# auggiemarignier/pxmcmc

Measured on AMD Instinct MI355X. Metric: MYULA samples/sec at L=256 synthesis, higher is better.
Workload: dtype f64

## Files before the change

include/pxmcmc_amd.h:

```cpp
#ifndef PXMCMC_AMD_H
#define PXMCMC_AMD_H

#include <stddef.h>
#include <stdint.h>

#ifdef __cplusplus
extern "C" {
#endif

typedef struct pxm_sht_plan_s* pxm_sht_plan_t;
typedef struct pxm_wav_plan_s* pxm_wav_plan_t;
typedef struct pxm_dwav_plan_s* pxm_dwav_plan_t;
typedef struct pxm_hwav_plan_s* pxm_hwav_plan_t;
typedef void* pxm_stream_t;

int pxm_version(void);
#ifdef PXM_NOISE_F64
#error "the -DPXM_NOISE_F64 build switch was removed: pass the flag PXM_NOISE_F64 per call (one library serves both precisions)"
#endif
#define PXM_NOISE_F64 16
int pxm_noise_bits(void);
int64_t pxm_host_check_address_ranges(int L, double B, int J_min, int spin, int max_chains, int what);
const char* pxm_last_error(void);
int pxm_device_count(void);

int pxm_capture_begin(void);
int pxm_capture_end(void);
int pxm_deferred_pending(void);
int pxm_tables_trim(void);

int pxm_j_max(int L, double B);
int pxm_wav_bandlimits(int L, double B, int J_min, int* bl_out, int cap);
int64_t pxm_wav_ncoefs(int L, double B, int J_min, int64_t* nscal_out);
int pxm_tiling_axisym(int L, double B, int J_min, double* kappa0, double* kappa);
int pxm_mw_ring_weights(int L, double* q);
int pxm_host_sht_tables(int L, int spin, int m, double* Binv, double* Afwd);
int pxm_host_rec_table(int L, int spin, int m, double* Brec);
int pxm_host_pfa511_tables(uint16_t* idx, double* b2);

int pxm_sht_plan_create(int L, int spin, int max_chains, unsigned flags, pxm_sht_plan_t* plan);
int pxm_sht_plan_destroy(pxm_sht_plan_t plan);
int pxm_sht_uses_recursion(pxm_sht_plan_t plan);
int pxm_rec_reduce_selftest(double* out128);
int pxm_sht_inverse(pxm_sht_plan_t plan, const void* flm, void* f, int C, pxm_stream_t stream);
int pxm_sht_forward(pxm_sht_plan_t plan, const void* f, void* flm, int C, pxm_stream_t stream);
// ... 170 lines not shown
```

pxmcmc_amd/_lib.py:

```python
import ctypes as C
import os

import torch

_HERE = os.path.dirname(os.path.abspath(__file__))
LIB_PATH = os.environ.get("PXM_LIB_PATH") or os.path.join(_HERE, "lib", "libpxmcmc_amd.so")

c_i64, c_u64, c_int, c_dbl, c_vp = C.c_int64, C.c_uint64, C.c_int, C.c_double, C.c_void_p

SIGNATURES = {
    "pxm_version": (c_int, []),
    "pxm_noise_bits": (c_int, []),
    "pxm_host_check_address_ranges": (c_i64, [c_int, c_dbl, c_int, c_int, c_int, c_int]),
    "pxm_last_error": (C.c_char_p, []),
    "pxm_device_count": (c_int, []),
    "pxm_capture_begin": (c_int, []),
    "pxm_capture_end": (c_int, []),
    "pxm_deferred_pending": (c_int, []),
    "pxm_tables_trim": (c_int, []),
    "pxm_wav_set_iter_counter": (c_int, [c_vp, c_vp]),
    "pxm_wav_release_iter_counter": (c_int, [c_vp, c_vp]),
    "pxm_wav_iter_counter_add": (c_int, [c_vp, c_u64, c_vp]),
    "pxm_wav_exact_dft_scales": (c_int, [c_vp]),
    "pxm_wav_status": (c_int, [c_vp, c_int, c_vp]),
    "pxm_sht_status": (c_int, [c_vp, c_int, c_vp]),
    "pxm_wav_profile_enable": (c_int, [c_vp, c_int]),
    "pxm_wav_profile_read": (c_int, [c_vp, c_vp, c_vp, c_vp, c_vp]),
    "pxm_wav_profile_read_launches": (c_int, [c_vp, c_vp, c_vp, c_vp, c_i64, c_vp]),
    "pxm_wav_profile_read_dft": (c_int, [c_vp, c_vp, c_vp, c_vp]),
    "pxm_wav_workspace_nonfinite": (c_i64, [c_vp, c_vp]),
    "pxm_reduce_scratch_doubles": (c_i64, [c_int]),
    "pxm_j_max": (c_int, [c_int, c_dbl]),
    "pxm_wav_bandlimits": (c_int, [c_int, c_dbl, c_int, c_vp, c_int]),
    "pxm_wav_ncoefs": (c_i64, [c_int, c_dbl, c_int, c_vp]),
    "pxm_tiling_axisym": (c_int, [c_int, c_dbl, c_int, c_vp, c_vp]),
    "pxm_mw_ring_weights": (c_int, [c_int, c_vp]),
# ... 159 lines not shown
```

pxmcmc_amd/csrc/sht_core.h:

```cpp
#pragma once
#include "common.h"

namespace pxm {

enum TableKind { TAB_INV = 0, TAB_FWD = 1, TAB_INV_ADJ = 2, TAB_FWD_ADJ = 3, TAB_GRAM = 4, TAB_KINDS = 5 };
inline bool kind_el_to_ring(int kind) { return kind == TAB_INV || kind == TAB_FWD_ADJ; }
inline bool kind_rows_are_el(int kind) { return kind == TAB_FWD || kind == TAB_INV_ADJ || kind == TAB_GRAM; }
inline bool kind_k_is_el(int kind) { return kind == TAB_INV || kind == TAB_FWD_ADJ || kind == TAB_GRAM; }

struct GemmTask {
  int64_t tab_off;
  int64_t rt_stride;
  int64_t x_off[4];
  int64_t y_off[4];
  int64_t x2_off[4];
  int64_t hd_off[4];
  int64_t ks_off[2];
  int64_t rs_off[2];
  int row_lo[2], row_hi[2];
  int k_beg, k_end;
  int row0;
  int n_rt;
  int nslab;
  double sign1;
  int m_unit;
  int hd_stride;
  int x_ncol, y_ncol;
};

struct GemmAffine {
  double ns = 0, wr = 0, wi = 0;
// ... 22 lines not shown
    p.launch_bytes.push_back(alg_bytes);
    p.launch_wgs.push_back(workgroups);
    ++p.used;
  }
};
int profiler_enable(Profiler* pr, int max_launches);
int profiler_read(Profiler::Pool* p, double* ms, int64_t* launches, double* bytes, double* flops,
                  double* per_launch_ms = nullptr, double* per_launch_bytes = nullptr, int64_t cap = 0,
                  int32_t* per_launch_wgs = nullptr);
void profiler_release(Profiler* pr);

struct GemmFuse {
  int64_t x2_base = -1;
  const double* rscale = nullptr;
  int row_lo = 0, row_hi = 1 << 30;
  int64_t hd_base = -1;
  int hd_stride = 0;
};

struct ShtTables {
  int L = 0, spin = 0, Rp = 0;
  bool paired = false;
  int n_m = 0;
  double* d_tab[TAB_KINDS] = {nullptr, nullptr, nullptr, nullptr, nullptr};
  size_t bytes[TAB_KINDS] = {0, 0, 0, 0, 0};
  std::vector<int64_t> m_off[TAB_KINDS];
  std::vector<int> k_beg[TAB_KINDS];
  int refs = 0;
  int m_of(int i) const { return paired ? i : i - (L - 1); }
};

int get_tables(int L, int spin, unsigned kinds_mask, ShtTables** out);
void retain_tables(ShtTables* T);
void release_tables(ShtTables* T);
int64_t tables_trim();

void append_gemm_tasks(const ShtTables& T, int kind, int ncol, int64_t x_base, int x_L, int x_Rp,
                       int64_t y_base, int y_L, int y_Rp, const double* kscale, int64_t scratch_off,
                       const double* ws_base, std::vector<GemmTask>& tasks, int el_lo = 0,
                       const GemmFuse& fuse = GemmFuse());
struct GemmSide {
  int64_t x_base, y_base;
  int x_L, x_Rp, y_L, y_Rp;
  const double* kscale;
  int el_lo;
  GemmFuse fuse;
  int x_ncol = 0, y_ncol = 0;
};

void append_gemm_tasks_packed(const ShtTables& T, int kind, int ncol, const GemmSide& side_a, const GemmSide* side_b,
                              int64_t scratch_off, const double* ws_base, std::vector<GemmTask>& tasks);
int launch_gemm_packed(const GemmTask* d_tasks, int n_tasks, int pk, int flags, const double* X, double* Y, int ncol, int col0,
                       double alg_bytes, double flops, hipStream_t stream, Profiler* prof = nullptr);
// ... 121 lines not shown
```

pxmcmc_amd/csrc/sht_gemm.hip:

```cpp
#include "../../include/pxmcmc_amd.h"
#include "sht_core.h"

#include <type_traits>

#include <hip/hip_ext.h>

#include <cstdlib>
#include <map>
#include <mutex>

namespace pxm {

typedef double d4 __attribute__((ext_vector_type(4)));

constexpr int KC = 16;
#define PXM_GEMM_MFMA(ACC, A, B) ACC = __builtin_amdgcn_mfma_f64_16x16x4f64(A, B, ACC, 0, 0, 0);
#ifdef PXM_GEMM_TRACE
__device__ unsigned long long* g_gemm_trace = nullptr;
extern "C" int pxm_debug_set_gemm_trace(unsigned long long* buf) {
  return hipMemcpyToSymbol(HIP_SYMBOL(g_gemm_trace), &buf, sizeof(buf)) == hipSuccess ? 0 : -1;
}
#endif
__device__ __forceinline__ double stage_add(double a, double b, bool on) { return a + (on ? b : 0.0); }
__device__ __forceinline__ double2 stage_add(double2 a, double2 b, bool on) { return double2{a.x + (on ? b.x : 0.0), a.y + (on ? b.y : 0.0)}; }
__device__ __forceinline__ double stage_scale(double a, double sc) { return a * sc; }
__device__ __forceinline__ double2 stage_scale(double2 a, double sc) { return double2{a.x * sc, a.y * sc}; }
template <int CT, int NSLAB>
struct GemmGeom {
  static constexpr int NCT = CT * NSLAB;
  static constexpr int COLS = 16 * NCT;
  static constexpr int PITCH = COLS + (COLS == 16 ? 0 : 16);
};
template <int CT, int NSLAB, int NW, int RT, int NSET, bool TWO, bool SK, int PK = 0>
__device__ __forceinline__ void sht_gemm_body(const GemmTask* __restrict__ tasks, const int bid,
                                              const double* __restrict__ X, double* __restrict__ Y, int ncol, int col0,
                                              const GemmAffine& aff, double (*xs)[KC][GemmGeom<CT, NSLAB>::PITCH]) {
  constexpr int NCT = CT * NSLAB;
  constexpr bool HOIST = TWO;
  constexpr int COLS = GemmGeom<CT, NSLAB>::COLS;
  constexpr int PITCH = GemmGeom<CT, NSLAB>::PITCH;
  constexpr int NT = 64 * NW;
  constexpr int VW = (KC * COLS / 2 >= NT) ? 2 : 1;
  constexpr int NV = KC * COLS / VW;
  constexpr int IT = (NV + NT - 1) / NT;
  const GemmTask t = tasks[bid];
  const int tid = threadIdx.x, lane = tid & 63;
  if (t.n_rt == 0) return;
  const int xn = PK ? t.x_ncol : ncol, yn = PK ? t.y_ncol : ncol;
#ifdef PXM_GEMM_TRACE
  const unsigned long long trace_t0 = wall_clock64();
  unsigned long long trace_t1 = 0, trace_t2 = 0;
  long long trace_c[5] = {0, 0, 0, 0, 0};
#define PXM_GEMM_CSTAMP(K) if (ch == 8) trace_c[K] = clock64();
#else
#define PXM_GEMM_CSTAMP(K)
#endif
  const int wave = __builtin_amdgcn_readfirstlane(tid >> 6);
  const int kq = lane >> 4, cl = lane & 15;
  const int n_my = min(RT, max(0, t.n_rt - RT * wave));
  const int nch = (t.k_end - t.k_beg) / KC;

  const double* sp[IT];
  const double* sp2[IT];
  const double* skp[IT];
  int so[IT];
  bool sv[IT];
#pragma unroll
  for (int i = 0; i < IT; ++i) {
    const int q0 = tid + NT * i;
    const int q = q0 % NV;
    const int kr = (q / (COLS / VW)) % KC, col = VW * (q % (COLS / VW));
// ... 140 lines not shown
    const int64_t yo = tasks[bid].y_off[live ? slab : 0];
    const int row_lo = grp ? t.row_lo[1] : t.row_lo[0], row_hi = grp ? t.row_hi[1] : t.row_hi[0];
#pragma unroll
    for (int r = 0; r < RT; ++r) {
      if (r >= n_my) continue;
      const int rowb = t.row0 + 16 * (RT * wave + r) + kq;
      double* yb = Y + yo + col0 + (cl % PK) + (int64_t)rowb * yn;
#pragma unroll
      for (int q = 0; q < 4; ++q) {
        const int row = rowb + 4 * q;
        const double rs = grp ? rsv[r][NGRP - 1][q] : rsv[r][0][q];
        if (live && row >= row_lo && row < row_hi) yb[(int64_t)(4 * q) * yn] = sgn * rs * acc[r][0][q];
      }
    }
  } else {
#pragma unroll
  for (int r = 0; r < RT; ++r) {
    if (r >= n_my) continue;
#pragma unroll
    for (int c = 0; c < NCT; ++c) {
      const int slab = c / CT, cin = 16 * (c % CT), grp = slab >> 1;
      const double sgn = (slab & 1) ? t.sign1 : 1.0;
      const int rowb = t.row0 + 16 * (RT * wave + r) + kq;
      double* yb = Y + t.y_off[slab] + col0 + cin + cl + (int64_t)rowb * ncol;
#pragma unroll
      for (int q = 0; q < 4; ++q) {
        const int row = rowb + 4 * q;
        double v = acc[r][c][q];
        if (aff.on) {
          const double u = aff.ns * v - hdv[r][slab][q];
          int lo = __double2loint(u), hi = __double2hiint(u);
          lo = __builtin_amdgcn_mov_dpp(lo, 0xB1, 0xF, 0xF, true);
          hi = __builtin_amdgcn_mov_dpp(hi, 0xB1, 0xF, 0xF, true);
          const double pu = __hiloint2double(hi, lo);
          v = (cl & 1) ? (aff.wr * u + aff.wi * pu) : (aff.wr * u - aff.wi * pu);
          if (col0 + cin + cl >= aff.ncol_live) v = 0.0;
        }
        if (row >= t.row_lo[grp] && row < t.row_hi[grp]) yb[(int64_t)(4 * q) * ncol] = sgn * rsv[r][grp][q] * v;
      }
    }
  }
  }
#ifdef PXM_GEMM_TRACE
  __syncthreads();
  if (tid == 0 && g_gemm_trace) {
    unsigned hw, xcc;
    asm volatile("s_getreg_b32 %0, hwreg(HW_REG_HW_ID)" : "=s"(hw));
    asm volatile("s_getreg_b32 %0, hwreg(HW_REG_XCC_ID)" : "=s"(xcc));
    const unsigned long long slot = atomicAdd(g_gemm_trace, 1ull);
    unsigned long long* r = g_gemm_trace + 8 + 8 * slot;
    r[0] = blockIdx.x; r[1] = gridDim.x; r[2] = trace_t0; r[3] = wall_clock64();
    r[4] = ((unsigned long long)(xcc & 0xf) << 32) | hw; r[5] = (unsigned long long)nch | ((unsigned long long)t.n_rt << 16) | ((unsigned long long)aff.on << 32);
    r[6] = trace_t1; r[7] = trace_t2;
    if (nch > 9) {
      const unsigned long long s2 = atomicAdd(g_gemm_trace + 1, 1ull);
      unsigned long long* q = g_gemm_trace + 8 + 8 * 8192 + 8 * s2;
      q[0] = nch; q[1] = trace_c[1] - trace_c[0]; q[2] = trace_c[2] - trace_c[1]; q[3] = trace_c[3] - trace_c[2];
      q[4] = trace_c[4] - trace_c[3]; q[5] = aff.on; q[6] = gridDim.x; q[7] = 0;
    }
  }
#endif
// ... 70 lines not shown
int check_gemm_task_ranges(const std::vector<GemmTask>& v, int nslab, int flags, int ncol, const double* ws_base,
                           const char* list_name) {
  int64_t n = 0;
  std::string why;
  auto bad = [&](size_t ti, const char* what, int col0) {
    set_error(std::string("GEMM task address range outside its buffer: list '") + list_name + "', task " + std::to_string(ti) +
              ", column group " + std::to_string(col0) + ", " + what + ": " + why);
    return -1;
  };
  auto ok = [&](int64_t lo, int64_t hi) {
    ++n;
    return lo <= hi && dev_range_ok(ws_base + lo, ws_base + hi + 1, &why);
  };
  const bool TWO = flags & 1, SK = flags & 2;
  for (size_t ti = 0; ti < v.size(); ++ti) {
    const GemmTask& t = v[ti];
    if (t.n_rt == 0) continue;
    const int nch = (t.k_end - t.k_beg) / KC;
    if (!ok(t.tab_off, t.tab_off + (int64_t)(t.n_rt - 1) * t.rt_stride + (int64_t)(2 * (nch - 1) + 1) * 128 + 127))
      return bad(ti, "ring-table stream", 0);
    for (int col0 = 0; col0 < ncol; col0 += 32) {
      const int CT = (ncol - col0 >= 32) ? 2 : 1;
      for (int slab = 0; slab < nslab; ++slab) {
        const int xn = t.x_ncol ? t.x_ncol : ncol, yn = t.y_ncol ? t.y_ncol : ncol;
        const int wx = std::min(16 * CT, xn), wy = std::min(16 * CT, yn);
        const int64_t lo = col0 + (int64_t)t.k_beg * xn, hi = col0 + wx - 1 + (int64_t)(t.k_end - 1) * xn;
        if (!ok(t.x_off[slab] + lo, t.x_off[slab] + hi)) return bad(ti, "operand staging", col0);
        if (TWO && t.x2_off[slab] && !ok(t.x2_off[slab] + lo, t.x2_off[slab] + hi)) return bad(ti, "second operand staging", col0);
        if (SK && t.ks_off[slab >> 1] && !ok(t.ks_off[slab >> 1] + t.k_beg, t.ks_off[slab >> 1] + t.k_end - 1))
          return bad(ti, "operand scale vector", col0);
        const int64_t r_lo = t.row0, r_hi = t.row0 + 16 * t.n_rt - 1;
        if (t.hd_off[slab] && !ok(t.hd_off[slab] + r_lo * t.hd_stride, t.hd_off[slab] + r_hi * t.hd_stride + 1))
          return bad(ti, "affine data term", col0);
        if (t.rs_off[slab >> 1] && !ok(t.rs_off[slab >> 1] + r_lo, t.rs_off[slab >> 1] + r_hi))
          return bad(ti, "per-row output scale", col0);
        const int64_t s_lo = std::max<int64_t>(r_lo, t.row_lo[slab >> 1]), s_hi = std::min<int64_t>(r_hi, (int64_t)t.row_hi[slab >> 1] - 1);
        if (s_lo <= s_hi && !ok(t.y_off[slab] + col0 + s_lo * yn, t.y_off[slab] + col0 + wy - 1 + s_hi * yn))
          return bad(ti, "result rows", col0);
      }
    }
  }
  ranges_checked_add(n);
  return 0;
}

int gemm_rows_per_task(int ncol) {
  (void)ncol;
// ... 67 lines not shown
    }
  } else {
    g.x_off[s1] = g.x_off[s0];
    g.y_off[s1] = g.y_off[s0];
  }
  g.ks_off[grp] = sd.kscale ? (sd.kscale - ws_base) : 0;
  g.rs_off[grp] = sd.fuse.rscale ? (sd.fuse.rscale - ws_base) : 0;
  g.row_lo[grp] = sd.fuse.row_lo;
  g.row_hi[grp] = sd.fuse.row_hi;
  g.x2_off[s0] = g.x2_off[s1] = 0;
  if (sd.fuse.x2_base >= 0) {
    g.x2_off[s0] = sd.fuse.x2_base + (int64_t)(m + sd.x_L - 1) * sd.x_Rp * xn;
    g.x2_off[s1] = (T.paired && m != 0) ? sd.fuse.x2_base + (int64_t)(-m + sd.x_L - 1) * sd.x_Rp * xn : g.x2_off[s0];
  }
  g.hd_off[s0] = g.hd_off[s1] = 0;
  g.hd_stride = sd.fuse.hd_stride > 0 ? sd.fuse.hd_stride : ncol;
  if (sd.fuse.hd_base >= 0) {
    g.hd_off[s0] = sd.fuse.hd_base + (int64_t)(m + sd.y_L - 1) * sd.y_Rp * g.hd_stride;
    g.hd_off[s1] = (T.paired && m != 0) ? sd.fuse.hd_base + (int64_t)(-m + sd.y_L - 1) * sd.y_Rp * g.hd_stride : g.hd_off[s0];
  }
  (void)kind;
}

static void append_tasks_impl(const ShtTables& T, int kind, int ncol, const GemmSide& side,
                              int64_t scratch_off, const double* ws_base, std::vector<GemmTask>& tasks) {
  const bool rows_el = kind_rows_are_el(kind), k_el = kind_k_is_el(kind);
  const int Rp = T.Rp;
  const int el_lo = side.el_lo;
  const int lo16 = round_down(std::max(el_lo, 0), 16);
  const int rpt = gemm_rows_per_task(ncol);
  for (int i = 0; i < T.n_m; ++i) {
    const int m = T.m_of(i);
    const int kb = T.k_beg[kind][i];
    const int start = std::max(kb, lo16);
    if (start >= Rp) continue;
    const int64_t rt_stride = (int64_t)((k_el ? Rp - kb : Rp) / 8) * 128;
    const int k_beg = k_el ? start : 0, k_end = Rp, row_beg = rows_el ? start : 0;
    const int64_t tab_skip = (rows_el ? (int64_t)((start - kb) / 16) * rt_stride : 0) + (k_el ? (int64_t)((start - kb) / 8) * 128 : 0);
    const int n_rt_total = (Rp - row_beg) / 16;
    for (int rt = 0; rt < n_rt_total; rt += rpt) {
      GemmTask g;
      g.m_unit = T.paired ? m : m + T.L - 1;
      g.tab_off = (T.d_tab[kind] + T.m_off[kind][i] + tab_skip + (int64_t)rt * rt_stride) - ws_base;
      g.rt_stride = rt_stride;
      for (int s = 0; s < 2; ++s) fill_side(g, s, T, kind, m, ncol, side, scratch_off, ws_base);
      g.nslab = T.paired ? 2 : 1;
      g.k_beg = k_beg;
      g.k_end = k_end;
      g.row0 = row_beg + 16 * rt;
      g.n_rt = std::min(rpt, n_rt_total - rt);
      g.sign1 = (kind == TAB_GRAM) ? 1.0 : ((m & 1) ? -1.0 : 1.0);
      g.x_ncol = side.x_ncol ? side.x_ncol : ncol;
      g.y_ncol = side.y_ncol ? side.y_ncol : ncol;
      tasks.push_back(g);
    }
  }
}

void append_gemm_tasks_packed(const ShtTables& T, int kind, int ncol, const GemmSide& side_a, const GemmSide* side_b,
                              int64_t scratch_off, const double* ws_base, std::vector<GemmTask>& tasks) {
  GemmSide sa = side_a;
  if (side_b) sa.el_lo = std::min(side_a.el_lo, side_b->el_lo);
  const size_t first = tasks.size();
  append_tasks_impl(T, kind, ncol, sa, scratch_off, ws_base, tasks);
  for (size_t i = first; i < tasks.size(); ++i) {
    GemmTask& g = tasks[i];
    const int m = T.paired ? g.m_unit : g.m_unit - (T.L - 1);
    fill_side(g, 0, T, kind, m, ncol, side_a, scratch_off, ws_base);
    fill_side(g, 1, T, kind, m, ncol, side_b ? *side_b : side_a, scratch_off, ws_base);
    g.nslab = side_b ? 4 : 2;
    g.x_ncol = side_a.x_ncol ? side_a.x_ncol : ncol;
    g.y_ncol = side_a.y_ncol ? side_a.y_ncol : ncol;
    if (!T.paired) {
      g.nslab = 1;
    }
  }
}
// ... 7 lines not shown

__global__ void k_build_fwd(const double* __restrict__ Bd, const double* __restrict__ Qd, double* __restrict__ Ad,
                            int Rp, int L, double scale, int m0, int spin) {
  const int i = blockIdx.z;
  const int el = blockIdx.x * 16 + threadIdx.x, t = blockIdx.y * 16 + threadIdx.y;
  const int m = m0 + i;
  const int par = ((m + spin) & 1) ? 1 : 0;
  const double* B = Bd + (int64_t)i * Rp * Rp;
  const double* Q = Qd + (int64_t)par * Rp * Rp;
  double acc = 0;
  for (int tp = 0; tp < L; ++tp) acc += B[(int64_t)tp * Rp + el] * Q[(int64_t)tp * Rp + t];
  Ad[(int64_t)i * Rp * Rp + (int64_t)el * Rp + t] = scale * acc;
}

__global__ void k_build_gram(const double* __restrict__ Bd, double* __restrict__ Gd, int Rp, int L) {
  const int i = blockIdx.z;
  const int r = blockIdx.x * 16 + threadIdx.x, c = blockIdx.y * 16 + threadIdx.y;
  const double* B = Bd + (int64_t)i * Rp * Rp;
  double acc = 0;
  for (int t = 0; t < L; ++t) acc += B[(int64_t)t * Rp + r] * B[(int64_t)t * Rp + c];
  Gd[(int64_t)i * Rp * Rp + (int64_t)r * Rp + c] = acc;
}

__global__ void k_tile_table(const double* __restrict__ D, double* __restrict__ out, int Rp, int row_beg,
                             int k_beg, int transposed) {
  const int nk2 = (Rp - k_beg) / 8;
  const int rt = blockIdx.y;
  const int kk2 = blockIdx.x;
  const int lane = threadIdx.x >> 1, h = threadIdx.x & 1;
  const int row = row_beg + 16 * rt + (lane & 15);
  const int k = k_beg + 8 * kk2 + 4 * h + (lane >> 4);
  const double v = transposed ? D[(int64_t)k * Rp + row] : D[(int64_t)row * Rp + k];
  out[((int64_t)rt * nk2 + kk2) * 128 + threadIdx.x] = v;
}

static std::mutex g_tab_mutex;
static std::map<std::pair<int, int>, ShtTables*> g_tab_cache;

static int build_kind(ShtTables& T, int kind, const double* d_B, const double* d_A, const double* d_G) {
  const int Rp = T.Rp;
  const bool rows_el = kind_rows_are_el(kind), k_el = kind_k_is_el(kind);
  T.m_off[kind].resize(T.n_m);
  T.k_beg[kind].resize(T.n_m);
  int64_t total = 0;
  for (int i = 0; i < T.n_m; ++i) {
    const int elmin = std::max(std::abs(T.m_of(i)), std::abs(T.spin));
    const int kb = round_down(elmin, 16);
    T.k_beg[kind][i] = kb;
    T.m_off[kind][i] = total;
    total += (int64_t)((rows_el ? Rp - kb : Rp) / 16) * ((k_el ? Rp - kb : Rp) / 8) * 128;
  }
  T.bytes[kind] = (size_t)total * sizeof(double);
  if (int rc = dev_alloc(&T.d_tab[kind], T.bytes[kind], "ring table")) return rc;
  if (dry_run()) return 0;
  for (int i = 0; i < T.n_m; ++i) {
    const int kb = T.k_beg[kind][i];
    const double* src;
    int transposed;
    if (kind == TAB_INV) { src = d_B; transposed = 0; }
    else if (kind == TAB_FWD_ADJ) { src = d_A; transposed = 1; }
    else if (kind == TAB_FWD) { src = d_A; transposed = 0; }
    else if (kind == TAB_INV_ADJ) { src = d_B; transposed = 1; }
    else { src = d_G; transposed = 0; }
    src += (int64_t)i * Rp * Rp;
    const int row_beg = rows_el ? kb : 0, k_beg = k_el ? kb : 0;
    dim3 grid((Rp - k_beg) / 8, (Rp - row_beg) / 16), block(128);
    if (grid.x == 0 || grid.y == 0) continue;
    hipLaunchKernelGGL(k_tile_table, grid, block, 0, 0, src, T.d_tab[kind] + T.m_off[kind][i], Rp, row_beg, k_beg,
                       transposed);
  }
  PXM_HIP(hipGetLastError());
  return 0;
}

int get_tables(int L, int spin, unsigned kinds_mask, ShtTables** out) {
  std::lock_guard<std::mutex> lock(g_tab_mutex);
  int dev = 15;
  if (!dry_run()) {
    PXM_HIP(hipGetDevice(&dev));
    PXM_REQUIRE(dev >= 0 && dev < 15, "get_tables: device index outside [0, 15)");
  }
  auto key = std::make_pair(L * 16 + dev, spin);
  ShtTables* T = nullptr;
  auto it = g_tab_cache.find(key);
  if (it != g_tab_cache.end()) T = it->second;
  else {
    T = new ShtTables();
    T->L = L;
    T->spin = spin;
    T->Rp = round_up(L, 16);
    T->paired = (spin == 0);
    T->n_m = T->paired ? L : 2 * L - 1;
// ... 10 lines not shown
      }
  } else if (missing) {
    const int Rp = T->Rp;
    const size_t dense = (size_t)T->n_m * Rp * Rp;
    std::vector<double> hB(dense, 0.0);
    const int m0 = T->paired ? 0 : -(L - 1);
    for (int i = 0; i < T->n_m; ++i) wigner_ring_table(L, spin, m0 + i, hB.data() + (size_t)i * Rp * Rp, Rp);
    double *d_B = nullptr, *d_A = nullptr, *d_Q = nullptr, *d_G = nullptr;
    PXM_HIP(hipMalloc(&d_B, dense * sizeof(double)));
    PXM_HIP(hipMemcpy(d_B, hB.data(), dense * sizeof(double), hipMemcpyHostToDevice));
    hB.clear();
    hB.shrink_to_fit();
    if (missing & ((1u << TAB_FWD) | (1u << TAB_FWD_ADJ))) {
      std::vector<double> hQ((size_t)2 * Rp * Rp, 0.0);
      quadrature_gram(L, +1, hQ.data(), Rp);
      quadrature_gram(L, -1, hQ.data() + (size_t)Rp * Rp, Rp);
      PXM_HIP(hipMalloc(&d_Q, hQ.size() * sizeof(double)));
      PXM_HIP(hipMemcpy(d_Q, hQ.data(), hQ.size() * sizeof(double), hipMemcpyHostToDevice));
      PXM_HIP(hipMalloc(&d_A, dense * sizeof(double)));
      dim3 grid(Rp / 16, Rp / 16, T->n_m), block(16, 16);
      hipLaunchKernelGGL(k_build_fwd, grid, block, 0, 0, d_B, d_Q, d_A, Rp, L, 2.0 * M_PI / (2 * L - 1), m0, spin);
      PXM_HIP(hipGetLastError());
    }
    if (missing & (1u << TAB_GRAM)) {
      PXM_HIP(hipMalloc(&d_G, dense * sizeof(double)));
      dim3 grid(Rp / 16, Rp / 16, T->n_m), block(16, 16);
      hipLaunchKernelGGL(k_build_gram, grid, block, 0, 0, d_B, d_G, Rp, L);
      PXM_HIP(hipGetLastError());
    }
    for (int k = 0; k < TAB_KINDS; ++k)
      if (missing >> k & 1u) {
        int rc = build_kind(*T, k, d_B, d_A, d_G);
        if (rc) return rc;
      }
    PXM_HIP(hipDeviceSynchronize());
    PXM_HIP(hipFree(d_B));
    if (d_A) PXM_HIP(hipFree(d_A));
    if (d_Q) PXM_HIP(hipFree(d_Q));
    if (d_G) PXM_HIP(hipFree(d_G));
  }
  *out = T;
  return 0;
}

void retain_tables(ShtTables* T) {
  std::lock_guard<std::mutex> lock(g_tab_mutex);
  if (T) ++T->refs;
// ... 27 lines not shown
```

pxmcmc_amd/csrc/tasklist.hip:

```cpp
#include "tasklist.h"

#include <algorithm>
#include <cstdlib>
#include <cstring>
#include <map>

namespace pxm {

static int64_t task_work(const GemmTask& a, int64_t fixed) { return (int64_t)(a.k_end - a.k_beg + fixed) * a.n_rt; }

static void order_xcd(std::vector<GemmTask>& v, int64_t fixed) {
  constexpr int NQ = 8;
  std::map<int64_t, int> unit_of;
  std::vector<std::vector<GemmTask>> units;
  for (const GemmTask& t : v) {
    auto it = unit_of.find(t.x_off[0]);
    if (it == unit_of.end()) {
      it = unit_of.emplace(t.x_off[0], (int)units.size()).first;
      units.emplace_back();
    }
    units[it->second].push_back(t);
  }
  std::vector<int64_t> uw(units.size(), 0);
  std::vector<int> idx(units.size());
// ... 33 lines not shown
  std::vector<int64_t> load(nbins, 0);
  for (const GemmTask& t : v) {
    int best = 0;
    for (int b = 1; b < nbins; ++b)
      if (load[b] < load[best] || (load[b] == load[best] && bins[b].size() < bins[best].size())) best = b;
    bins[best].push_back(t);
    load[best] += task_work(t, fixed);
  }
  std::vector<GemmTask> ordered;
  ordered.reserve(v.size());
  for (size_t r = 0;; ++r) {
    bool any = false;
    for (int b = 0; b < nbins; ++b)
      if (r < bins[b].size()) {
        ordered.push_back(bins[b][r]);
        any = true;
      }
    if (!any) break;
  }
  v.swap(ordered);
}

void order_tasks(std::vector<GemmTask>& v, const std::string& order) {
  const int64_t fixed = order == "xcd" ? 32 : 0;
  std::stable_sort(v.begin(), v.end(), [&](const GemmTask& a, const GemmTask& b) { return task_work(a, fixed) > task_work(b, fixed); });
  if (order == "xcd" && !v.empty()) order_xcd(v, fixed);
  else if (order == "bins" && (int)v.size() > 256) order_bins(v, fixed);
}

int upload_tasks(std::vector<GemmTask> v, bool paired, TaskList* out, std::vector<int> bls, int ncol, const double* ws_base,
                 const char* name, std::vector<int> los, int pk, std::vector<char> tab_shared) {
  tab_shared.resize(bls.size(), 0);
  los.resize(bls.size(), 0);
  out->pk = pk;
  out->tab_shared = tab_shared;
  out->bls = bls;
  out->los = los;
  const char* order_env = getenv("PXM_GEMM_ORDER");
  order_tasks(v, order_env ? order_env : (v.size() > 2048 ? "xcd" : "bins"));
  out->n = (int)v.size();
  out->paired = paired;
  out->nslab = pk ? 4 : (paired ? 2 : 1);
  for (const GemmTask& t : v) {
    PXM_REQUIRE(t.n_rt >= 0 && t.n_rt <= 8 && t.row0 >= 0 && t.row0 % 16 == 0 && t.k_beg >= 0 && t.k_beg % 16 == 0 &&
                    (t.n_rt == 0 || (t.k_end > t.k_beg && (t.k_end - t.k_beg) % 16 == 0)),
                "upload_tasks: malformed GEMM task");
    out->mfma_units += (double)t.n_rt * ((t.k_end - t.k_beg) / 4) * (pk ? 1 : t.nslab);
    for (int sl = 0; sl < 4; ++sl)
      if (t.x2_off[sl]) out->flags |= 1;
    if (t.ks_off[0] || t.ks_off[1]) out->flags |= 2;
  }
  if (v.empty()) return 0;
  if (int rc = check_gemm_task_ranges(v, out->nslab, out->flags, ncol, ws_base, name)) return rc;
  if (int rc = dev_alloc(&out->d, v.size() * sizeof(GemmTask), "GEMM task list")) return rc;
  return dev_upload(out->d, v.data(), v.size() * sizeof(GemmTask));
}

double tasklist_bytes(const TaskList& tl, int cg) {
  double bytes = 0;
  for (size_t i = 0; i < tl.bls.size(); ++i) {
    const double Ld = tl.bls[i];
    if (tl.gram) bytes += tl.gram_table_bytes + 3 * 16.0 * cg * Ld * Ld + 16.0 * Ld * Ld;
    else bytes += gemm_alg_bytes(tl.bls[i], tl.paired, cg, tl.los[i]);
    if (!tl.gram && tl.pk && tl.tab_shared[i]) bytes -= gemm_table_bytes(tl.bls[i], tl.paired, tl.los[i]);
  }
  return bytes;
}

int run_tasks(const TaskList& tl, const double* X, double* Y, int ncol, int C, hipStream_t st, const GemmAffine& aff,
              Profiler* prof) {
  note_stream(st);
  if (tl.pk)
    return launch_gemm_packed(tl.d, tl.n, tl.pk, tl.flags, X, Y, ncol, 0, tasklist_bytes(tl, C), tl.mfma_units * 2048.0, st, prof);
  for (int col0 = 0; col0 < ncol; col0 += 32) {
// ... 20 lines not shown
```

pxmcmc_amd/csrc/wav_plan.hip:

```cpp
#include "wav_plan.h"

#include <cmath>
#include <memory>
#include <mutex>

using namespace pxm;

struct SideOverride {
  const int64_t* g = nullptr;
  int g_ncol = 0;
  const WlAttach* h = nullptr;
};
static GemmSide wav_side(const pxm_wav_plan_s* p, int s, int which, const SideOverride& ov = SideOverride()) {
  const int L = p->L, b = p->bl[s], Rb = round_up(b, 16);
  const int64_t G = ov.g ? *ov.g : p->offG[s];
  GemmSide g;
  const bool ring_is_x = which == 0 || which == 3;
  if (ov.g && ov.g_ncol) (ring_is_x ? g.x_ncol : g.y_ncol) = ov.g_ncol;
  if (ov.h) (ring_is_x ? g.y_ncol : g.x_ncol) = ov.h->ncol_h;
  g.el_lo = p->el_lo_s[s];
  g.fuse = GemmFuse();
  g.kscale = nullptr;
  const int cls = (s == 0) ? 1 : ((s - 1) & 1);
  const int64_t hcls = ov.h ? (cls ? ov.h->offHBn : ov.h->offHAn) : (cls ? p->offHB : p->offHA);
// ... 169 lines not shown
  if ((rc = wav_level_list(p, TAB_FWD, p->offGL, p->offHL, GemmFuse(), &p->ana_fwd, "analysis forward at L"))) return rc;
  if ((rc = wav_level_list(p, TAB_FWD_ADJ, p->offHA, p->offGL, sum2, &p->anadj_fwdadj, "analysis-adjoint forward-adjoint at L"))) return rc;
  p->lane_of.assign(p->nsc, -1);
  SidePool* sp = nullptr;
  if ((rc = side_pool(&sp))) return rc;
  for (int i = 0; i < p->nside; ++i) {
    p->side[i] = sp->side[i];
    p->ev_join[i] = sp->ev_join[i];
  }
  p->ev_fork = sp->ev_fork;
  int k = 0;
  for (int s = p->nsc - 1; s >= 0; --s)
    if (p->bl[s] < L) p->lane_of[s] = (k++) % p->nside;
  std::vector<const DftPlan*> dp;
  for (int s = 0; s < p->nsc; ++s) dp.push_back(&p->dft[s]);
  if ((rc = dft_group_create(dp, p->offG, p->coef_off, p->ncol, p->ws, &p->dft_group)) < 0) return rc;
  *plan = guard.release();
  return 0;
}

int pxm::wav_make_gram_lists(pxm_wav_plan_s* p) {
  if (p->gram.d) return 0;
  int rc;
  if ((rc = get_tables(p->L, p->spin, 1u << TAB_GRAM, &p->TL))) return rc;
  wav_hold(p, p->TL);
  std::vector<GemmTask> v;
  GemmFuse fz;
  fz.x2_base = p->offHB;
  fz.hd_base = p->offHDc;
  fz.hd_stride = 2;
  append_gemm_tasks(*p->TL, TAB_GRAM, p->ncol, p->offHA, p->L, p->Rp, p->offHL, p->L, p->Rp, nullptr, p->offS, p->ws, v, 0, fz);
  if ((rc = upload_tasks(v, p->TL->paired, &p->gram, {p->L}, p->ncol, p->ws, "Gram step"))) return rc;
  p->gram.gram = true;
  p->gram.gram_table_bytes = (double)p->TL->bytes[TAB_GRAM];
  return wav_level_list(p, TAB_INV_ADJ, p->offGD, p->offHD, GemmFuse(), &p->adj_invadj_D, "inverse-adjoint of the data rings");
}

namespace pxm {
__global__ void k_iter_add(uint64_t* c, uint64_t inc) { *c += inc; }

__global__ void k_count_nonfinite(const double* __restrict__ x, int64_t n, unsigned long long* cnt) {
  unsigned long long c = 0;
  for (int64_t i = blockIdx.x * (int64_t)blockDim.x + threadIdx.x; i < n; i += (int64_t)gridDim.x * blockDim.x)
    if (!isfinite(x[i])) ++c;
  if (c) atomicAdd(cnt, c);
}
}

extern "C" {

int pxm_wav_plan_create(int L, double B, int J_min, int max_chains, unsigned flags, pxm_wav_plan_t* plan) {
  (void)flags;
  return wav_plan_create_impl("pxm_wav_plan_create", L, B, J_min, 0, max_chains, plan);
}

int pxm_wav_plan_create_spin(int L, double B, int J_min, int spin, int max_chains, unsigned flags, pxm_wav_plan_t* plan) {
  (void)flags;
// ... 99 lines not shown
  std::lock_guard<std::mutex> lock(mu);
  PXM_REQUIRE(!capture_in_progress(), "pxm_host_check_address_ranges: not during a stream capture");
  set_dry_run(true);
  ranges_checked_reset();
  int rc = 0;
  if (what & 1) {
    pxm_sht_plan_t sp = nullptr;
    rc = pxm_sht_plan_create(L, spin, max_chains, 0, &sp);
    if (sp) pxm_sht_plan_destroy(sp);
  }
  if (!rc && (what & 2)) {
    pxm_wav_plan_t wp = nullptr;
    const int wspin = (what & 8) ? spin : 0;
    rc = pxm_wav_plan_create_spin(L, B, J_min, wspin, max_chains, 0, &wp);
    if (!rc) rc = wav_make_gram_lists(wp);
    if (!rc && (what & 4) && L >= 3 && wspin == 0) rc = pxm_wav_wl_attach(wp, nullptr, nullptr, (int64_t)L * (2 * L - 1));
    if (wp) pxm_wav_plan_destroy(wp);
  }
  tables_trim();
  set_dry_run(false);
  return rc ? -1 : ranges_checked();
}

}
```

Baseline: 114,800.

## Split spin-0 Gram tables by ring parity into two half-size blocks

```diff
diff --git a/include/pxmcmc_amd.h b/include/pxmcmc_amd.h
--- a/include/pxmcmc_amd.h
+++ b/include/pxmcmc_amd.h
@@ -21,6 +21,7 @@
 #define PXM_NOISE_F64 16
 int pxm_noise_bits(void);
 int64_t pxm_host_check_address_ranges(int L, double B, int J_min, int spin, int max_chains, int what);
+int64_t pxm_host_gram_table_bytes(int L, double B, int J_min, int spin, int max_chains);
 const char* pxm_last_error(void);
 int pxm_device_count(void);
 
diff --git a/pxmcmc_amd/_lib.py b/pxmcmc_amd/_lib.py
--- a/pxmcmc_amd/_lib.py
+++ b/pxmcmc_amd/_lib.py
@@ -12,6 +12,7 @@
     "pxm_version": (c_int, []),
     "pxm_noise_bits": (c_int, []),
     "pxm_host_check_address_ranges": (c_i64, [c_int, c_dbl, c_int, c_int, c_int, c_int]),
+    "pxm_host_gram_table_bytes": (c_i64, [c_int, c_dbl, c_int, c_int, c_int]),
     "pxm_last_error": (C.c_char_p, []),
     "pxm_device_count": (c_int, []),
     "pxm_capture_begin": (c_int, []),
diff --git a/pxmcmc_amd/csrc/sht_core.h b/pxmcmc_amd/csrc/sht_core.h
--- a/pxmcmc_amd/csrc/sht_core.h
+++ b/pxmcmc_amd/csrc/sht_core.h
@@ -3,10 +3,11 @@
 
 namespace pxm {
 
-enum TableKind { TAB_INV = 0, TAB_FWD = 1, TAB_INV_ADJ = 2, TAB_FWD_ADJ = 3, TAB_GRAM = 4, TAB_KINDS = 5 };
+enum TableKind { TAB_INV = 0, TAB_FWD = 1, TAB_INV_ADJ = 2, TAB_FWD_ADJ = 3, TAB_GRAM = 4, TAB_GRAM_SPLIT = 5, TAB_KINDS = 6 };
 inline bool kind_el_to_ring(int kind) { return kind == TAB_INV || kind == TAB_FWD_ADJ; }
-inline bool kind_rows_are_el(int kind) { return kind == TAB_FWD || kind == TAB_INV_ADJ || kind == TAB_GRAM; }
-inline bool kind_k_is_el(int kind) { return kind == TAB_INV || kind == TAB_FWD_ADJ || kind == TAB_GRAM; }
+inline bool kind_is_gram(int kind) { return kind == TAB_GRAM || kind == TAB_GRAM_SPLIT; }
+inline bool kind_rows_are_el(int kind) { return kind == TAB_FWD || kind == TAB_INV_ADJ || kind_is_gram(kind); }
+inline bool kind_k_is_el(int kind) { return kind == TAB_INV || kind == TAB_FWD_ADJ || kind_is_gram(kind); }
 
 struct GemmTask {
   int64_t tab_off;
@@ -75,13 +76,23 @@
   int L = 0, spin = 0, Rp = 0;
   bool paired = false;
   int n_m = 0;
-  double* d_tab[TAB_KINDS] = {nullptr, nullptr, nullptr, nullptr, nullptr};
-  size_t bytes[TAB_KINDS] = {0, 0, 0, 0, 0};
+  double* d_tab[TAB_KINDS] = {};
+  size_t bytes[TAB_KINDS] = {};
   std::vector<int64_t> m_off[TAB_KINDS];
   std::vector<int> k_beg[TAB_KINDS];
+  std::vector<int64_t> odd_off;
+  std::vector<int> odd_k_beg;
   int refs = 0;
   int m_of(int i) const { return paired ? i : i - (L - 1); }
 };
+
+inline bool gram_can_split(const ShtTables& T) { return T.paired && T.Rp % 32 == 0; }
+constexpr int GEMM_TASK_FIXED_STEPS = 32;
+inline int gram_half_k_beg(int m, int par) { return round_down((m - par + 1) / 2, 16); }
+inline bool gram_order_splits(int Rp, int m) {
+  auto work = [](int n, int kb) { return (n - kb) / 16 * (n - kb + GEMM_TASK_FIXED_STEPS); };
+  return work(Rp / 2, gram_half_k_beg(m, 0)) + work(Rp / 2, gram_half_k_beg(m, 1)) < work(Rp, round_down(m, 16));
+}
 
 int get_tables(int L, int spin, unsigned kinds_mask, ShtTables** out);
 void retain_tables(ShtTables* T);
diff --git a/pxmcmc_amd/csrc/sht_gemm.hip b/pxmcmc_amd/csrc/sht_gemm.hip
--- a/pxmcmc_amd/csrc/sht_gemm.hip
+++ b/pxmcmc_amd/csrc/sht_gemm.hip
@@ -46,7 +46,7 @@
   const GemmTask t = tasks[bid];
   const int tid = threadIdx.x, lane = tid & 63;
   if (t.n_rt == 0) return;
-  const int xn = PK ? t.x_ncol : ncol, yn = PK ? t.y_ncol : ncol;
+  const int xn = (PK || TWO) ? t.x_ncol : ncol, yn = (PK || TWO) ? t.y_ncol : ncol;
 #ifdef PXM_GEMM_TRACE
   const unsigned long long trace_t0 = wall_clock64();
   unsigned long long trace_t1 = 0, trace_t2 = 0;
@@ -233,7 +233,7 @@
       const int slab = c / CT, cin = 16 * (c % CT), grp = slab >> 1;
       const double sgn = (slab & 1) ? t.sign1 : 1.0;
       const int rowb = t.row0 + 16 * (RT * wave + r) + kq;
-      double* yb = Y + t.y_off[slab] + col0 + cin + cl + (int64_t)rowb * ncol;
+      double* yb = Y + t.y_off[slab] + col0 + cin + cl + (int64_t)rowb * yn;
 #pragma unroll
       for (int q = 0; q < 4; ++q) {
         const int row = rowb + 4 * q;
@@ -247,7 +247,7 @@
           v = (cl & 1) ? (aff.wr * u + aff.wi * pu) : (aff.wr * u - aff.wi * pu);
           if (col0 + cin + cl >= aff.ncol_live) v = 0.0;
         }
-        if (row >= t.row_lo[grp] && row < t.row_hi[grp]) yb[(int64_t)(4 * q) * ncol] = sgn * rsv[r][grp][q] * v;
+        if (row >= t.row_lo[grp] && row < t.row_hi[grp]) yb[(int64_t)(4 * q) * yn] = sgn * rsv[r][grp][q] * v;
       }
     }
   }
@@ -364,7 +364,7 @@
     for (int col0 = 0; col0 < ncol; col0 += 32) {
       const int CT = (ncol - col0 >= 32) ? 2 : 1;
       for (int slab = 0; slab < nslab; ++slab) {
-        const int xn = t.x_ncol ? t.x_ncol : ncol, yn = t.y_ncol ? t.y_ncol : ncol;
+        const int xn = ((TWO || nslab == 4) && t.x_ncol) ? t.x_ncol : ncol, yn = ((TWO || nslab == 4) && t.y_ncol) ? t.y_ncol : ncol;
         const int wx = std::min(16 * CT, xn), wy = std::min(16 * CT, yn);
         const int64_t lo = col0 + (int64_t)t.k_beg * xn, hi = col0 + wx - 1 + (int64_t)(t.k_end - 1) * xn;
         if (!ok(t.x_off[slab] + lo, t.x_off[slab] + hi)) return bad(ti, "operand staging", col0);
@@ -478,37 +478,59 @@
   (void)kind;
 }
 
+static void append_block_tasks(const ShtTables& T, int kind, int ncol, const GemmSide& side, int64_t scratch_off,
+                               const double* ws_base, std::vector<GemmTask>& tasks, int m, const double* tab, int kb, int n,
+                               int par) {
+  const bool rows_el = kind_rows_are_el(kind), k_el = kind_k_is_el(kind);
+  const int lo16 = round_down(std::max(side.el_lo, 0), 16);
+  const int rpt = gemm_rows_per_task(ncol);
+  const int start = std::max(kb, lo16);
+  if (start >= n) return;
+  const int64_t rt_stride = (int64_t)((k_el ? n - kb : n) / 8) * 128;
+  const int k_beg = k_el ? start : 0, k_end = n, row_beg = rows_el ? start : 0;
+  const int64_t tab_skip = (rows_el ? (int64_t)((start - kb) / 16) * rt_stride : 0) + (k_el ? (int64_t)((start - kb) / 8) * 128 : 0);
+  const int n_rt_total = (n - row_beg) / 16;
+  for (int rt = 0; rt < n_rt_total; rt += rpt) {
+    GemmTask g;
+    g.m_unit = T.paired ? m : m + T.L - 1;
+    g.tab_off = (tab + tab_skip + (int64_t)rt * rt_stride) - ws_base;
+    g.rt_stride = rt_stride;
+    for (int s = 0; s < 2; ++s) fill_side(g, s, T, kind, m, ncol, side, scratch_off, ws_base);
+    g.nslab = T.paired ? 2 : 1;
+    g.k_beg = k_beg;
+    g.k_end = k_end;
+    g.row0 = row_beg + 16 * rt;
+    g.n_rt = std::min(rpt, n_rt_total - rt);
+    g.sign1 = kind_is_gram(kind) ? 1.0 : ((m & 1) ? -1.0 : 1.0);
+    g.x_ncol = side.x_ncol ? side.x_ncol : ncol;
+    g.y_ncol = side.y_ncol ? side.y_ncol : ncol;
+    if (par >= 0) {
+      for (int s = 0; s < 4; ++s) {
+        g.x_off[s] += par * g.x_ncol;
+        g.y_off[s] += par * g.y_ncol;
+        if (g.x2_off[s]) g.x2_off[s] += par * g.x_ncol;
+        if (g.hd_off[s]) g.hd_off[s] += par * g.hd_stride;
+      }
+      g.x_ncol *= 2;
+      g.y_ncol *= 2;
+      g.hd_stride *= 2;
+      for (int grp = 0; grp < 2; ++grp) g.row_lo[grp] = round_down(m, 16) / 2;
+    }
+    tasks.push_back(g);
+  }
+}
+
 static void append_tasks_impl(const ShtTables& T, int kind, int ncol, const GemmSide& side,
                               int64_t scratch_off, const double* ws_base, std::vector<GemmTask>& tasks) {
-  const bool rows_el = kind_rows_are_el(kind), k_el = kind_k_is_el(kind);
-  const int Rp = T.Rp;
-  const int el_lo = side.el_lo;
-  const int lo16 = round_down(std::max(el_lo, 0), 16);
-  const int rpt = gemm_rows_per_task(ncol);
   for (int i = 0; i < T.n_m; ++i) {
     const int m = T.m_of(i);
+    const double* tab = T.d_tab[kind] + T.m_off[kind][i];
     const int kb = T.k_beg[kind][i];
-    const int start = std::max(kb, lo16);
-    if (start >= Rp) continue;
-    const int64_t rt_stride = (int64_t)((k_el ? Rp - kb : Rp) / 8) * 128;
-    const int k_beg = k_el ? start : 0, k_end = Rp, row_beg = rows_el ? start : 0;
-    const int64_t tab_skip = (rows_el ? (int64_t)((start - kb) / 16) * rt_stride : 0) + (k_el ? (int64_t)((start - kb) / 8) * 128 : 0);
-    const int n_rt_total = (Rp - row_beg) / 16;
-    for (int rt = 0; rt < n_rt_total; rt += rpt) {
-      GemmTask g;
-      g.m_unit = T.paired ? m : m + T.L - 1;
-      g.tab_off = (T.d_tab[kind] + T.m_off[kind][i] + tab_skip + (int64_t)rt * rt_stride) - ws_base;
-      g.rt_stride = rt_stride;
-      for (int s = 0; s < 2; ++s) fill_side(g, s, T, kind, m, ncol, side, scratch_off, ws_base);
-      g.nslab = T.paired ? 2 : 1;
-      g.k_beg = k_beg;
-      g.k_end = k_end;
-      g.row0 = row_beg + 16 * rt;
-      g.n_rt = std::min(rpt, n_rt_total - rt);
-      g.sign1 = (kind == TAB_GRAM) ? 1.0 : ((m & 1) ? -1.0 : 1.0);
-      g.x_ncol = side.x_ncol ? side.x_ncol : ncol;
-      g.y_ncol = side.y_ncol ? side.y_ncol : ncol;
-      tasks.push_back(g);
+    if (kind == TAB_GRAM_SPLIT && T.odd_off[i] >= 0) {
+      append_block_tasks(T, kind, ncol, side, scratch_off, ws_base, tasks, m, tab, kb, T.Rp / 2, 0);
+      append_block_tasks(T, kind, ncol, side, scratch_off, ws_base, tasks, m, T.d_tab[kind] + T.odd_off[i], T.odd_k_beg[i], T.Rp / 2, 1);
+    } else {
+      append_block_tasks(T, kind, ncol, side, scratch_off, ws_base, tasks, m, tab, kb, T.Rp, -1);
     }
   }
 }
@@ -562,14 +584,18 @@
   Gd[(int64_t)i * Rp * Rp + (int64_t)r * Rp + c] = acc;
 }
 
-__global__ void k_tile_table(const double* __restrict__ D, double* __restrict__ out, int Rp, int row_beg,
-                             int k_beg, int transposed) {
-  const int nk2 = (Rp - k_beg) / 8;
+__global__ void k_tile_table(const double* __restrict__ D, double* __restrict__ out, int Rp, int n, int row_beg,
+                             int k_beg, int transposed, int par) {
+  const int nk2 = (n - k_beg) / 8;
   const int rt = blockIdx.y;
   const int kk2 = blockIdx.x;
   const int lane = threadIdx.x >> 1, h = threadIdx.x & 1;
-  const int row = row_beg + 16 * rt + (lane & 15);
-  const int k = k_beg + 8 * kk2 + 4 * h + (lane >> 4);
+  int row = row_beg + 16 * rt + (lane & 15);
+  int k = k_beg + 8 * kk2 + 4 * h + (lane >> 4);
+  if (par >= 0) {
+    row = 2 * row + par;
+    k = 2 * k + par;
+  }
   const double v = transposed ? D[(int64_t)k * Rp + row] : D[(int64_t)row * Rp + k];
   out[((int64_t)rt * nk2 + kk2) * 128 + threadIdx.x] = v;
 }
@@ -577,7 +603,52 @@
 static std::mutex g_tab_mutex;
 static std::map<std::pair<int, int>, ShtTables*> g_tab_cache;
 
+static int build_gram_split(ShtTables& T, const double* d_G) {
+  const int kind = TAB_GRAM_SPLIT, Rp = T.Rp, Rh = Rp / 2;
+  PXM_REQUIRE(gram_can_split(T), "build_gram_split: the parity split needs spin-0 tables and Rp % 32 == 0");
+  T.m_off[kind].assign(T.n_m, 0);
+  T.k_beg[kind].assign(T.n_m, 0);
+  T.odd_off.assign(T.n_m, -1);
+  T.odd_k_beg.assign(T.n_m, 0);
+  int64_t total = 0;
+  for (int m = 0; m < T.n_m; ++m) {
+    if (m == 0 || !gram_order_splits(Rp, m)) {
+      const int kb = round_down(m, 16);
+      T.k_beg[kind][m] = kb;
+      T.m_off[kind][m] = total;
+      total += (int64_t)((Rp - kb) / 16) * ((Rp - kb) / 8) * 128;
+      continue;
+    }
+    for (int par = 0; par < 2; ++par) {
+      const int kb = gram_half_k_beg(m, par);
+      (par ? T.odd_k_beg[m] : T.k_beg[kind][m]) = kb;
+      (par ? T.odd_off[m] : T.m_off[kind][m]) = total;
+      total += (int64_t)((Rh - kb) / 16) * ((Rh - kb) / 8) * 128;
+    }
+  }
+  T.bytes[kind] = (size_t)total * sizeof(double);
+  if (int rc = dev_alloc(&T.d_tab[kind], T.bytes[kind], "ring table")) return rc;
+  if (dry_run()) return 0;
+  for (int m = 0; m < T.n_m; ++m) {
+    const double* src = d_G + (int64_t)m * Rp * Rp;
+    if (T.odd_off[m] < 0) {
+      const int kb = T.k_beg[kind][m];
+      hipLaunchKernelGGL(k_tile_table, dim3((Rp - kb) / 8, (Rp - kb) / 16), dim3(128), 0, 0, src, T.d_tab[kind] + T.m_off[kind][m],
+                         Rp, Rp, kb, kb, 0, -1);
+      continue;
+    }
+    for (int par = 0; par < 2; ++par) {
+      const int kb = par ? T.odd_k_beg[m] : T.k_beg[kind][m];
+      hipLaunchKernelGGL(k_tile_table, dim3((Rh - kb) / 8, (Rh - kb) / 16), dim3(128), 0, 0, src,
+                         T.d_tab[kind] + (par ? T.odd_off[m] : T.m_off[kind][m]), Rp, Rh, kb, kb, 0, par);
+    }
+  }
+  PXM_HIP(hipGetLastError());
+  return 0;
+}
+
 static int build_kind(ShtTables& T, int kind, const double* d_B, const double* d_A, const double* d_G) {
+  if (kind == TAB_GRAM_SPLIT) return build_gram_split(T, d_G);
   const int Rp = T.Rp;
   const bool rows_el = kind_rows_are_el(kind), k_el = kind_k_is_el(kind);
   T.m_off[kind].resize(T.n_m);
@@ -606,8 +677,8 @@
     const int row_beg = rows_el ? kb : 0, k_beg = k_el ? kb : 0;
     dim3 grid((Rp - k_beg) / 8, (Rp - row_beg) / 16), block(128);
     if (grid.x == 0 || grid.y == 0) continue;
-    hipLaunchKernelGGL(k_tile_table, grid, block, 0, 0, src, T.d_tab[kind] + T.m_off[kind][i], Rp, row_beg, k_beg,
-                       transposed);
+    hipLaunchKernelGGL(k_tile_table, grid, block, 0, 0, src, T.d_tab[kind] + T.m_off[kind][i], Rp, Rp, row_beg, k_beg,
+                       transposed, -1);
   }
   PXM_HIP(hipGetLastError());
   return 0;
@@ -664,7 +735,7 @@
       hipLaunchKernelGGL(k_build_fwd, grid, block, 0, 0, d_B, d_Q, d_A, Rp, L, 2.0 * M_PI / (2 * L - 1), m0, spin);
       PXM_HIP(hipGetLastError());
     }
-    if (missing & (1u << TAB_GRAM)) {
+    if (missing & ((1u << TAB_GRAM) | (1u << TAB_GRAM_SPLIT))) {
       PXM_HIP(hipMalloc(&d_G, dense * sizeof(double)));
       dim3 grid(Rp / 16, Rp / 16, T->n_m), block(16, 16);
       hipLaunchKernelGGL(k_build_gram, grid, block, 0, 0, d_B, d_G, Rp, L);
diff --git a/pxmcmc_amd/csrc/tasklist.hip b/pxmcmc_amd/csrc/tasklist.hip
--- a/pxmcmc_amd/csrc/tasklist.hip
+++ b/pxmcmc_amd/csrc/tasklist.hip
@@ -79,7 +79,7 @@
 }
 
 void order_tasks(std::vector<GemmTask>& v, const std::string& order) {
-  const int64_t fixed = order == "xcd" ? 32 : 0;
+  const int64_t fixed = order == "xcd" ? GEMM_TASK_FIXED_STEPS : 0;
   std::stable_sort(v.begin(), v.end(), [&](const GemmTask& a, const GemmTask& b) { return task_work(a, fixed) > task_work(b, fixed); });
   if (order == "xcd" && !v.empty()) order_xcd(v, fixed);
   else if (order == "bins" && (int)v.size() > 256) order_bins(v, fixed);
@@ -107,6 +107,9 @@
       if (t.x2_off[sl]) out->flags |= 1;
     if (t.ks_off[0] || t.ks_off[1]) out->flags |= 2;
   }
+  if (!pk && !(out->flags & 1))
+    for (const GemmTask& t : v)
+      PXM_REQUIRE(t.n_rt == 0 || (t.x_ncol == ncol && t.y_ncol == ncol), "upload_tasks: a streaming list with a row pitch of its own");
   if (v.empty()) return 0;
   if (int rc = check_gemm_task_ranges(v, out->nslab, out->flags, ncol, ws_base, name)) return rc;
   if (int rc = dev_alloc(&out->d, v.size() * sizeof(GemmTask), "GEMM task list")) return rc;
diff --git a/pxmcmc_amd/csrc/wav_plan.hip b/pxmcmc_amd/csrc/wav_plan.hip
--- a/pxmcmc_amd/csrc/wav_plan.hip
+++ b/pxmcmc_amd/csrc/wav_plan.hip
@@ -215,17 +215,19 @@
 int pxm::wav_make_gram_lists(pxm_wav_plan_s* p) {
   if (p->gram.d) return 0;
   int rc;
-  if ((rc = get_tables(p->L, p->spin, 1u << TAB_GRAM, &p->TL))) return rc;
+  const char* split_env = getenv("PXM_GRAM_SPLIT");
+  const int kind = (gram_can_split(*p->TL) && !(split_env && atoi(split_env) == 0)) ? TAB_GRAM_SPLIT : TAB_GRAM;
+  if ((rc = get_tables(p->L, p->spin, 1u << kind, &p->TL))) return rc;
   wav_hold(p, p->TL);
   std::vector<GemmTask> v;
   GemmFuse fz;
   fz.x2_base = p->offHB;
   fz.hd_base = p->offHDc;
   fz.hd_stride = 2;
-  append_gemm_tasks(*p->TL, TAB_GRAM, p->ncol, p->offHA, p->L, p->Rp, p->offHL, p->L, p->Rp, nullptr, p->offS, p->ws, v, 0, fz);
+  append_gemm_tasks(*p->TL, kind, p->ncol, p->offHA, p->L, p->Rp, p->offHL, p->L, p->Rp, nullptr, p->offS, p->ws, v, 0, fz);
   if ((rc = upload_tasks(v, p->TL->paired, &p->gram, {p->L}, p->ncol, p->ws, "Gram step"))) return rc;
   p->gram.gram = true;
-  p->gram.gram_table_bytes = (double)p->TL->bytes[TAB_GRAM];
+  p->gram.gram_table_bytes = (double)p->TL->bytes[kind];
   return wav_level_list(p, TAB_INV_ADJ, p->offGD, p->offHD, GemmFuse(), &p->adj_invadj_D, "inverse-adjoint of the data rings");
 }
 
@@ -371,4 +373,19 @@
   return rc ? -1 : ranges_checked();
 }
 
-}
+int64_t pxm_host_gram_table_bytes(int L, double B, int J_min, int spin, int max_chains) {
+  static std::mutex mu;
+  std::lock_guard<std::mutex> lock(mu);
+  PXM_REQUIRE(!capture_in_progress(), "pxm_host_gram_table_bytes: not during a stream capture");
+  set_dry_run(true);
+  pxm_wav_plan_t wp = nullptr;
+  int rc = pxm_wav_plan_create_spin(L, B, J_min, spin, max_chains, 0, &wp);
+  if (!rc) rc = wav_make_gram_lists(wp);
+  const int64_t bytes = rc ? -1 : (int64_t)wp->gram.gram_table_bytes;
+  if (wp) pxm_wav_plan_destroy(wp);
+  tables_trim();
+  set_dry_run(false);
+  return bytes;
+}
+
+}
```

After: 116,600, median of 6. 1.6% higher.
